# tier4/icp_rust

Hardware: AMD Instinct MI355X
Metric: ICP iterations/sec on 1M-pt 3D pair (higher is better)
Workload: dtype f64

## Files before the change

icp_rust_amd/csrc/api.hip:

```cpp
#include <dlfcn.h>
#include <fcntl.h>
#include <sys/mman.h>
#include <unistd.h>

#include <cfloat>
#include <chrono>
#include <cstdio>
#include <cstring>
#include <atomic>
#include <map>
#include <mutex>
#include <new>

#include "api_internal.hpp"

using namespace icp;
using namespace icp::api;

namespace icp {
namespace api {
int map_hip(hipError_t e) {
  switch (e) {
    case hipSuccess: return ICP_OK;
    case hipErrorOutOfMemory: return ICP_OUT_OF_MEMORY;
    case hipErrorNoDevice:
    case hipErrorInvalidDevice:
    case hipErrorInsufficientDriver:
    case hipErrorNotInitialized: return ICP_NO_DEVICE;
    default: return ICP_HIP_ERROR;
  }
}
}
}

namespace {

template <typename Tp>
hipError_t grow(Tp *&p, size_t count) {
  if (p) {
    hipError_t e = hipFree(p);
    p = nullptr;
    if (e != hipSuccess) return e;
  }
  return hipMalloc(&p, (count ? count : 1) * sizeof(Tp));
}

void free_ctx(GnCtx &c) {
  (void)hipFree(c.d_rx);
  (void)hipFree(c.d_ry);
  (void)hipFree(c.d_hist);
  (void)hipFree(c.d_cand);
  (void)hipFree(c.d_ctl);
  (void)hipFree(c.d_sel);
  (void)hipFree(c.d_scal);
  (void)hipFree(c.d_partials);
  (void)hipFree(c.d_whist);
  (void)hipFree(c.d_wstate);
  (void)hipFree(c.d_wmed);
  (void)hipFree(c.d_wring);
  (void)hipFree(c.d_bkt);
  (void)hipFree(c.d_bkt_dir);
  (void)hipFree(c.d_wjoin);
  if (c.h_res) (void)hipHostFree(c.h_res);
}

void free_workspace(Workspace &w) {
  (void)hipFree(w.d_src);
  (void)hipFree(w.d_a);
  (void)hipFree(w.d_b);
  (void)hipFree(w.d_a2);
  (void)hipFree(w.d_b2);
  (void)hipFree(w.d_a3);
  (void)hipFree(w.d_b3);
  (void)hipFree(w.d_ahead);
  (void)hipFree(w.d_idx);
  (void)hipFree(w.d_idx_slot);
  (void)hipFree(w.d_sa);
  (void)hipFree(w.d_sb);
  if (w.h_whist) (void)hipHostFree(w.h_whist);
  if (w.h_tiny) (void)hipHostFree(w.h_tiny);
  (void)hipFree(w.d_rlist);
  (void)hipFree(w.d_rlist_len);
  (void)hipFree(w.d_part_d);
  (void)hipFree(w.d_part_i);
  free_loop_inbox(w);
  free_loop_plan(w.loop_plan);
  (void)hipFree(w.d_loop_ctl);
  (void)hipFree(w.d_loop_hist);
  (void)hipFree(w.d_loop_part);
  if (w.h_loop_res) (void)hipHostFree(w.h_loop_res);
  free_ctx(w);
  free_ctx(w.alt);
  if (w.spec_stream) {
    (void)hipStreamSynchronize(w.spec_stream);
    (void)hipStreamDestroy(w.spec_stream);
  }
  w = Workspace();
}

hipError_t alloc_ctx(GnCtx &c, hipStream_t s) {
  hipError_t e;
  const size_t hist_bytes = (size_t)kSelRoles * kSelProblems * kSelBins * sizeof(uint32_t);
  if ((e = hipMalloc(&c.d_hist, hist_bytes)) != hipSuccess) return e;
  if ((e = hipMemsetAsync(c.d_hist, 0, hist_bytes, s)) != hipSuccess) return e;
  if ((e = hipMalloc(&c.d_cand, (size_t)2 * kSelProblems * kSelCap * sizeof(unsigned long long))) != hipSuccess) return e;
  if ((e = hipMalloc(&c.d_ctl, sizeof(SelCtl))) != hipSuccess) return e;
  if ((e = hipMemsetAsync(c.d_ctl, 0, sizeof(SelCtl), s)) != hipSuccess) return e;
  if ((e = hipMalloc(&c.d_sel, 2 * kSelProblems * sizeof(SelState))) != hipSuccess) return e;
  if ((e = hipMalloc(&c.d_scal, sizeof(GnScalars))) != hipSuccess) return e;
  if ((e = hipMalloc(&c.d_partials, (size_t)(kTreeMaxBlocks + 1) * (kNSum + 1) * sizeof(double))) != hipSuccess) return e;
  const size_t whist_bytes = ((size_t)2 * kWinBins + kShardStatusWords) * sizeof(uint32_t);
  if ((e = hipMalloc(&c.d_whist, whist_bytes)) != hipSuccess) return e;
  if ((e = hipMemsetAsync(c.d_whist, 0, whist_bytes, s)) != hipSuccess) return e;
  if ((e = hipMalloc(&c.d_wstate, sizeof(WinState))) != hipSuccess) return e;
  if ((e = hipMemsetAsync(c.d_wstate, 0, sizeof(WinState), s)) != hipSuccess) return e;
  if ((e = hipMalloc(&c.d_wmed, (size_t)2 * kWinCapMed * sizeof(double))) != hipSuccess) return e;
  if ((e = hipMalloc(&c.d_wring, (size_t)2 * kWinCapRing * sizeof(double))) != hipSuccess) return e;
  if ((e = hipMalloc(&c.d_bkt, (size_t)kReduceMaxBlocks * kBktStage * sizeof(double))) != hipSuccess) return e;
  if ((e = hipMalloc(&c.d_bkt_dir, (size_t)kReduceMaxBlocks * kBktDir * sizeof(unsigned short))) != hipSuccess) return e;
  if ((e = hipMalloc(&c.d_wjoin, sizeof(WinJoin))) != hipSuccess) return e;
  if ((e = hipMemsetAsync(c.d_wjoin, 0, sizeof(WinJoin), s)) != hipSuccess) return e;
  if ((e = hipHostMalloc(&c.h_res, sizeof(GnResult), hipHostMallocCoherent)) != hipSuccess) return e;
  memset(c.h_res, 0, sizeof(GnResult));
  return hipSuccess;
}

}

namespace icp {

namespace {
using PushFn = int (*)(const char *);
using PopFn = int (*)();
PushFn g_roctx_push = nullptr;
PopFn g_roctx_pop = nullptr;
std::once_flag g_roctx_once;
void roctx_lookup() {
  for (const char *lib : {"librocprofiler-sdk-roctx.so", "librocprofiler-sdk-roctx.so.1", "libroctx64.so", "libroctx64.so.4"}) {
    void *hnd = dlopen(lib, RTLD_LAZY | RTLD_GLOBAL);
    if (!hnd) continue;
    g_roctx_push = reinterpret_cast<PushFn>(dlsym(hnd, "roctxRangePushA"));
    g_roctx_pop = reinterpret_cast<PopFn>(dlsym(hnd, "roctxRangePop"));
    if (g_roctx_push && g_roctx_pop) return;
    g_roctx_push = nullptr;
    g_roctx_pop = nullptr;
  }
}
}
Range::Range(const char *name) {
  std::call_once(g_roctx_once, roctx_lookup);
  if (g_roctx_push) (void)g_roctx_push(name);
}
Range::~Range() {
  if (g_roctx_pop) (void)g_roctx_pop();
}

hipError_t ensure_workspace(icp_handle *h, size_t n, bool need_src) {
  Workspace &w = h->ws;
  hipError_t e;
  if (!w.d_hist) {
    if ((e = alloc_ctx(w, h->stream)) != hipSuccess) return e;
    if ((e = alloc_ctx(w.alt, h->stream)) != hipSuccess) return e;
    int prio_least = 0, prio_greatest = 0;
    (void)hipDeviceGetStreamPriorityRange(&prio_least, &prio_greatest);
    if ((e = hipStreamCreateWithPriority(&w.spec_stream, hipStreamNonBlocking, prio_greatest)) != hipSuccess) return e;
    if ((e = hipMalloc(&w.d_ahead, sizeof(AheadPose))) != hipSuccess) return e;
    if ((e = hipMemsetAsync(w.d_ahead, 0, sizeof(AheadPose), h->stream)) != hipSuccess) return e;
    if ((e = hipStreamSynchronize(h->stream)) != hipSuccess) return e;
  }
  if (n > w.cap_n) {
    if ((e = hipStreamSynchronize(h->stream)) != hipSuccess) return e;
    if ((e = hipStreamSynchronize(w.spec_stream)) != hipSuccess) return e;
    size_t cap = n + n / 8;
    (void)hipFree(w.d_src);
    w.d_src = nullptr;
    if ((e = grow(w.d_a, cap * 2)) != hipSuccess) return e;
    if ((e = grow(w.d_b, cap * 2)) != hipSuccess) return e;
    if ((e = grow(w.d_a2, cap * 2)) != hipSuccess) return e;
    if ((e = grow(w.d_b2, cap * 2)) != hipSuccess) return e;
    if ((e = grow(w.d_a3, cap * 2)) != hipSuccess) return e;
    if ((e = grow(w.d_b3, cap * 2)) != hipSuccess) return e;
    if ((e = grow(w.d_rx, cap)) != hipSuccess) return e;
    if ((e = grow(w.d_ry, cap)) != hipSuccess) return e;
    if ((e = grow(w.alt.d_rx, cap)) != hipSuccess) return e;
    if ((e = grow(w.alt.d_ry, cap)) != hipSuccess) return e;
    if ((e = grow(w.d_idx, cap)) != hipSuccess) return e;
    if ((e = grow(w.d_idx_slot, cap)) != hipSuccess) return e;
    w.cap_n = cap;
  }
  if (need_src && !w.d_src) {
    if ((e = hipMalloc(&w.d_src, (w.cap_n ? w.cap_n : 1) * 3 * sizeof(double))) != hipSuccess) return e;
  }
  return hipSuccess;
}

}

extern "C" const char *icp_status_string(int s) {
  switch (s) {
    case ICP_OK: return "ok";
    case ICP_NONE: return "none (the reference returns None)";
    case ICP_EMPTY_DST: return "empty dst (the reference panics on index.unwrap())";
    case ICP_NAN_INPUT: return "NaN residual (the reference panics on partial_cmp().unwrap())";
    case ICP_BAD_ARGUMENT: return "bad argument";
    case ICP_NO_DEVICE: return "no usable HIP device (there is no CPU fallback)";
    case ICP_HIP_ERROR: return "HIP error";
    case ICP_OUT_OF_MEMORY: return "out of device memory";
    case ICP_RETRY_REPLICATED: return "sharded evaluation: evaluate this one on the gathered pairs";
    case ICP_RETRY_SHARDED: return "sharded evaluation: the window missed; again with the refined window";
    default: return "unknown status";
  }
}

extern "C" int icp_abi_version(void) { return ICP_ABI_VERSION; }

extern "C" int icp_device_pci_bus_id(int device, char out[64]) {
  if (!out) return ICP_BAD_ARGUMENT;
  out[0] = 0;
  if (hipDeviceGetPCIBusId(out, 64, device) != hipSuccess) {
    (void)hipGetLastError();
    return ICP_NO_DEVICE;
  }
  return ICP_OK;
}

extern "C" int icp_device_count(void) {
  int n = 0;
  if (hipGetDeviceCount(&n) != hipSuccess) return 0;
  return n;
}

extern "C" void icp_transform_new(const double p[3], icp_pose *out) { *out = transform_new(p); }
extern "C" void icp_transform_from_rt(const double r[4], const double t[2], icp_pose *out) {
  *out = icp_pose{r[0], r[1], r[2], r[3], t[0], t[1]};
}
extern "C" void icp_transform_identity(icp_pose *out) { *out = transform_identity(); }
extern "C" void icp_transform_apply(const icp_pose *T, const double p[2], double out[2]) {
  double o[2];
  transform_apply(*T, p, o);
  out[0] = o[0];
  out[1] = o[1];
}
extern "C" void icp_transform_inverse(const icp_pose *T, icp_pose *out) { *out = transform_inverse(*T); }
extern "C" void icp_transform_mul(const icp_pose *l, const icp_pose *r, icp_pose *out) {
  *out = transform_mul(*l, *r);
}
extern "C" void icp_se2_exp(const double p[3], double m[9]) { se2_exp(p, m); }
extern "C" void icp_se2_log(const double m[9], double p[3]) { se2_log(m, p); }
// ... 753 lines not shown
          if (on_eval_stream) {
            h->stream = first_stream;
            h->ws.swap_ctx();
          }
          return map_hip(he);
        }
      }
      {
        const int kind_now = it == 0 ? first_kind : (it == 1 ? second_kind : 2);
        if (!(it == 0 && first_pre_launched)) adopt_pool_hint(h->ws, kind_now);
      }
      const int rc = (it == 1 && !hook_first)
                         ? wgn_step(h, d_a, d_b, n, T, delta, &err, [&] { return second_eval_hook(T); }, false, second_kind)
                         : wgn_step(h, d_a, d_b, n, T, delta, &err, it == 0 && first_pre_launched,
                                    it == 0 ? first_kind : (it == 1 ? second_kind : 2));
      if (on_eval_stream) {
        h->stream = first_stream;
        h->ws.swap_ctx();
      }
      if (rc == ICP_NONE) break;
      if (rc != ICP_OK) return rc;
      if ((delta[0] * delta[0] + delta[1] * delta[1]) + delta[2] * delta[2] < ICP_DELTA_NORM_THRESHOLD)
        break;
      if (err > prev_error) break;
      prev_error = err;
      T = transform_mul(transform_new(delta), T);
      ++applied;
    }
  }
  *out = T;
  if (inner_iters) *inner_iters = applied;
  return ICP_OK;
}

extern "C" int icp_estimate_transform_device(icp_handle *h, const double *d_a, const double *d_b, size_t n,
                                             icp_pose *out, uint32_t *inner_iters) {
  if (!h || !out || (n > 0 && (!d_a || !d_b)) || n >= 0xffffffffull) return ICP_BAD_ARGUMENT;
  if (input_size_ok(n)) {
    HIP_TRY(hipSetDevice(h->device));
    HIP_TRY(ensure_workspace(h, n, false));
  }
  return estimate_transform_loop(h, d_a, d_b, n, out, inner_iters, [](const Pose &) { return hipSuccess; });
}

int icp::api::estimate_transform_on_pairs(icp_handle *h, const double *d_a, const double *d_b, size_t n, Pose *out,
                                          uint32_t *inner_iters, int first_kind, int second_kind) {
  return estimate_transform_loop(h, d_a, d_b, n, out, inner_iters, [](const Pose &) { return hipSuccess; }, nullptr,
                                 false, false, first_kind, second_kind);
}

extern "C" int icp_estimate_device(icp_handle *h, const double *d_src, size_t n, const icp_pose *init,
                                   size_t max_iter, icp_pose *out, uint32_t *d_last_idx,
                                   uint32_t *inner_iters) {
  if (!h || !init || !out || (n > 0 && !d_src) || n >= 0xffffffffull) return ICP_BAD_ARGUMENT;
  HIP_TRY(hipSetDevice(h->device));
  HIP_TRY(ensure_workspace(h, n, false));
  struct Quiesce {
    icp_handle *h;
    ~Quiesce() {
      h->ws.bkt_pair_launched = h->ws.alt.bkt_pair_launched = false;
      (void)hipStreamSynchronize(h->stream);
      if (h->ws.spec_stream) (void)hipStreamSynchronize(h->ws.spec_stream);
      h->qsort.valid = false;
      h->qsort.have_prev = false;
      h->qsort.slot_order = false;
    }
  } quiesce_on_exit{h};
  h->qsort.fold_n = 0;
  if (n > 0 && max_iter > 0 && h->m > 0) {
    int tiny_status = -1;
    HIP_TRY(launch_tiny_estimate(h, d_src, n, *init, max_iter, out, d_last_idx, inner_iters, &tiny_status));
    if (tiny_status == 0) {
      ++h->ws.tiny_calls;
      return ICP_OK;
    }
    if (tiny_status == 3) return ICP_NAN_INPUT;
  }
  static const bool no_spec = getenv("ICP_NO_SPECULATION") != nullptr;
  Workspace &w = h->ws;
  const bool loop_ok = gn_loop_applies(n);
  const bool two_streams = !no_spec && h->stream == h->own_stream;
  Pose T = *init;
  if (max_iter > 0) {
    const int prc = icp_prepare_source_device(h, d_src, n, init);
    if (prc != ICP_OK) return prc;
  }
  const bool slot = h->qsort.valid && h->qsort.src == d_src && h->qsort.n == n && (long)n > kGridCoopMaxN;
  h->qsort.slot_order = slot;
  if (slot) h->qsort.fold_n = n;
  uint32_t *const idx_target = slot ? w.d_idx_slot : d_last_idx;
  double *A[3] = {w.d_a, w.d_a2, w.d_a3}, *B[3] = {w.d_b, w.d_b2, w.d_b3};
  int cur = 0;
  bool spec_valid = false, pre_valid = false, first_pre_launched = false;
  const bool can_ahead = two_streams && resolved_nn_mode(h) == ICP_NN_GRID;
  bool ahead_issued = false;
  bool hooked_first = false;
  Pose spec_pose = T;
  uint32_t prev_inner = w.last_inner != 0xffffffffu ? w.last_inner : w.hint_last_inner;
  hipStream_t search_stream = h->stream;
  for (size_t it = 0; it < max_iter; ++it) {
    if (spec_valid && memcmp(&spec_pose, &T, sizeof(Pose)) == 0) {
      cur = (cur + 1) % 3;
      ++w.spec_hits;
      first_pre_launched = pre_valid;
    } else {
      first_pre_launched = false;
      ahead_issued = false;
      if (spec_valid) ++w.spec_misses;
      uint32_t *idx_out = (it + 1 == max_iter && d_last_idx) ? idx_target : nullptr;
      const int rc = icp_correspond_device(h, d_src, n, &T, A[cur], B[cur], idx_out);
      if (rc != ICP_OK) return rc;
    }
    spec_valid = false;
    pre_valid = false;
    const bool device_loop = loop_ok && !first_pre_launched && !(two_streams && prev_inner == 1) && loop_allowed(w);
    const bool speculate = !device_loop && !no_spec && n > 0 && h->m > 0 && it + 1 < max_iter && prev_inner == 1;
    auto launch_spec = [&](const Pose &T1) -> hipError_t {
      spec_pose = transform_mul(T1, T);
      uint32_t *idx_out = (it + 2 == max_iter && d_last_idx) ? idx_target : nullptr;
      const int nxt = (cur + 1) % 3, nxt2 = (cur + 2) % 3;
      spec_valid = true;
      pre_valid = false;
      hipStream_t eval_stream = h->stream;
      h->stream = search_stream;
      hipError_t e = hipSuccess;
      const bool have_search = ahead_issued && w.ahead_seen_valid && memcmp(&w.ahead_seen_pose, &spec_pose, sizeof(Pose)) == 0;
      if (ahead_issued && (have_search || w.ahead_seen_valid)) ++(have_search ? w.ahead_hits : w.ahead_misses);
      ahead_issued = false;
      if (!have_search) e = launch_nn(h, d_src, n, &spec_pose, A[nxt], B[nxt], idx_out);
      if (e == hipSuccess && two_streams) {
        WinParams P;
        w.swap_ctx();
        if (w.gn_dirty) {
          e = launch_sel_init(h, n);
          w.gn_dirty = false;
        }
        if (e == hipSuccess && window_usable(h, n, &P, 0)) {
          ++w.win_tried;
          const bool go_ahead = can_ahead && it + 2 < max_iter;
          WinParams P2;
          const int kind2 = it == 0 ? 4 : 1;
          bool pair = hooked_first && w.bkt_off == 0 && !w.alt.gn_dirty && !w.alt.bkt_pair_launched && bkt_fits(n, P);
          if (pair) {
            adopt_pool_hint(w, kind2);
            pair = window_usable(h, n, &P2, kind2) && bkt_fits(n, P2);
          }
          if (pair) {
            ++w.win_tried;
            e = launch_bkt_pair(h, h->stream, w, A[nxt], B[nxt], P, go_ahead, spec_pose, w.alt, A[cur], B[cur], T1, P2, n);
          } else {
            w.ahead_on = go_ahead;
            w.ahead_outer = spec_pose;
            e = launch_weighted_gn_win(h, A[nxt], B[nxt], n, transform_identity(), P);
            w.ahead_on = false;
          }
          pre_valid = true;
          if (e == hipSuccess && go_ahead) {
            uint32_t *idx_out2 = (it + 3 == max_iter && d_last_idx) ? idx_target : nullptr;
            e = launch_nn_grid_ahead(h, d_src, n, w.d_ahead, A[nxt2], B[nxt2], idx_out2, &ahead_issued);
          }
        }
        w.swap_ctx();
      }
      h->stream = eval_stream;
      return e;
    };
    auto hook = [&](const Pose &T1) -> hipError_t { return speculate ? launch_spec(T1) : hipSuccess; };
// ... 254 lines not shown
```

icp_rust_amd/csrc/common.hpp:

```cpp
#pragma once
#include <hip/hip_runtime.h>

#include <cstddef>
#include <cstdint>
#include <cstdlib>
#include <utility>
#include <vector>

#include "pose.hpp"

namespace icp {


struct Range {
  explicit Range(const char *name);
  ~Range();
  Range(const Range &) = delete;
  Range &operator=(const Range &) = delete;
};

constexpr int kReduceThreads = 512;
constexpr int kReduceMaxBlocks = 256;
constexpr int kTreeMaxBlocks = 2048;
constexpr int kShardMaxWorld = 16;
// ... 68 lines not shown
  unsigned med_cnt[2];
  unsigned ring_inner[2];
  unsigned ring_cnt[2];
  double med_lo[2], med_hi[2];
  double ring_lo[2], ring_hi[2];
  unsigned list_cnt[4][32];
};

struct WinJoinDim {
  double med, sig;
  double tot[10];
  unsigned flags;
  unsigned pad[7];
};
static_assert(sizeof(WinJoinDim) == 128, "a line per dimension");
struct WinJoin {
  unsigned ticket;
  unsigned pad[31];
  WinJoinDim dim[2];
};

struct GnResult {
  double acc[kNAcc + 1];
  double sigma[2];
  double median[2];
  int nan_flag;
  int overflow;
  unsigned seq;
  unsigned pad;
  unsigned status[4];
  Pose next_pose;
  int next_valid;
  int pad2;
};

struct AheadPose {
  Pose T;
  int valid;
  int pad;
};

struct GnCtx {
  double *d_rx = nullptr;
  double *d_ry = nullptr;
  uint32_t *d_hist = nullptr;
  unsigned long long *d_cand = nullptr;
  SelCtl *d_ctl = nullptr;
  SelState *d_sel = nullptr;
  GnScalars *d_scal = nullptr;
  double *d_partials = nullptr;
  GnResult *h_res = nullptr;
  unsigned seq = 0;
  bool gn_dirty = true;
  uint32_t *d_whist = nullptr;
  WinState *d_wstate = nullptr;
  double *d_wmed = nullptr;
  double *d_wring = nullptr;
  double *d_bkt = nullptr;
  unsigned short *d_bkt_dir = nullptr;
  WinJoin *d_wjoin = nullptr;
  bool bkt_pair_launched = false;
};

struct Workspace : GnCtx {
  GnCtx alt;
  void swap_ctx() { std::swap(static_cast<GnCtx &>(*this), alt); }
  size_t cap_n = 0;
  double *d_src = nullptr;
  double *d_a = nullptr;
  double *d_b = nullptr;
  double *d_a2 = nullptr;
  double *d_b2 = nullptr;
  double *d_a3 = nullptr;
  double *d_b3 = nullptr;
  AheadPose *d_ahead = nullptr;
  bool ahead_on = false;
  Pose ahead_outer;
  bool ahead_seen_valid = false;
  Pose ahead_seen_pose;
  unsigned long long ahead_hits = 0, ahead_misses = 0;
  unsigned long long spec_hits = 0, spec_misses = 0;
  uint32_t last_inner = 0xffffffffu;
  hipStream_t spec_stream = nullptr;
  uint32_t *d_idx = nullptr;
  uint32_t *d_idx_slot = nullptr;
  double *d_sa = nullptr, *d_sb = nullptr;
  uint32_t *h_whist = nullptr;
  void *h_tiny = nullptr;
  unsigned long long tiny_calls = 0, tiny_evals = 0, tiny_sorted = 0;
  double *d_rlist = nullptr;
  unsigned *d_rlist_len = nullptr;
  size_t cap_part = 0;
  double *d_part_d = nullptr;
  uint32_t *d_part_i = nullptr;
  bool win_valid = false;
  bool win_wide = false;
  double win_med[2] = {0., 0.}, win_sigma[2] = {0., 0.};
  struct WinPred {
    bool valid = false, wide = false;
    double med[2] = {0., 0.}, sigma[2] = {0., 0.};
  };
  WinPred win_kind[5];
  WinPred hint_kind[5];
  uint32_t hint_last_inner = 0xffffffffu;
  static bool kind_has_slot(int kind) { return kind == 0 || kind == 1 || kind == 3 || kind == 4; }
  unsigned long long win_tried = 0, win_missed = 0, short_evals = 0, radix_evals = 0;
  unsigned long long bkt_evals = 0, bkt_misses = 0;
  unsigned long long fixed_point_skips = 0;
  unsigned bkt_off = 0;
  void *d_loop_ctl = nullptr, *h_loop_res = nullptr;
  uint32_t *d_loop_hist = nullptr;
  double *d_loop_part = nullptr;
  unsigned loop_seq = 0;
  bool loop_off = false;
  unsigned long long loop_launches = 0, loop_evals = 0, loop_handbacks = 0, loop_timeouts = 0;
  void *d_loop_inbox = nullptr;
  int loop_inbox_kind = 0;
  void *loop_inbox_host = nullptr;
  char loop_shm_name[64] = {0};
  unsigned loop_probe_gen = 0;
  unsigned loop_off_calls = 0;
  void *loop_peers[kShardMaxWorld] = {};
  int loop_rank = -1, loop_world = 0;
  void *loop_plan = nullptr;
  unsigned pipe_gen = 0;
  unsigned long long pipe_iters = 0, pipe_handbacks = 0, pipe_gave_up = 0;
  unsigned pipe_off = 0;
};

struct GridParams {
  double lo[3];
  double hi[3];
  double h[3], inv_h[3];
  int n[3];
  int fx;
  double scale;
  float ext;
  int f32_ok;
  float hf[3], ihf[3], nm1f[3];
};

struct GridPoint {
  float x, y, z;
  uint32_t idx;
};

struct Grid {
  bool built = false;
  GridParams p;
  uint32_t ncell = 0;
  uint32_t *d_start = nullptr;
  GridPoint *d_pts = nullptr;
  size_t cap_start = 0, cap_pts = 0;
  uint32_t *t_cell_of = nullptr, *t_cnt = nullptr, *t_btot = nullptr;
  size_t cap_tcell = 0, cap_tcnt = 0, cap_tbtot = 0;
  double *t_part = nullptr;
  uint32_t *d_rcell = nullptr, *d_rcell2 = nullptr, *d_start2 = nullptr, *t_shift = nullptr, *t_cell_new = nullptr;
  GridPoint *d_pts2 = nullptr;
  size_t cap_rcell = 0, cap_rcell2 = 0, cap_start2 = 0, cap_pts2 = 0, cap_shift = 0, cap_cell_new = 0;
  size_t m_full = 0;
  bool rcell_valid = false;
  unsigned long long appends_moved = 0, appends_rebuilt = 0;
  unsigned long long crops_moved = 0, crops_rebuilt = 0;
  uint32_t *d_flag = nullptr;
};

constexpr int kShardStatusWords = 4;
constexpr unsigned kGridPad = 8;

struct ShardCandHeader {
  unsigned cnt[4];
  unsigned fail;
  unsigned pad[11];
};
struct ShardPtrs {
  const unsigned char *p[kShardMaxWorld];
};

struct PrevMatch {
  double x, y, z;
  uint32_t idx, pad;
};

struct QuerySort {
  bool valid = false;
  bool slot_order = false;
  bool identity = false;
  bool presorted = false;
  bool sort_only = false;
  size_t fold_n = 0;
  const double *src = nullptr;
  size_t n = 0, cap = 0;
  uint32_t *d_cell_of = nullptr;
  uint32_t *d_perm = nullptr;
  void *d_tmp = nullptr;
  size_t cap_tmp = 0;
  bool have_prev = false;
  PrevMatch *d_prev = nullptr;
  double *d_sorted = nullptr;
  bool have_certs = false, have_pose = false, have_pose_before = false;
  double decay_r = 0., decay_t = 0.;
  Pose last_pose;
  uint32_t *d_cert_lists = nullptr;
  unsigned *d_cert_ctr = nullptr, *last_cert_ctr = nullptr;
  unsigned cert_seq = 0;
  unsigned long long cert_searches = 0;
};

hipError_t stable_sort_cells(const uint32_t *keys_in, uint32_t *perm_out, unsigned n, unsigned bits, void *&tmp, size_t &cap_tmp,
                             hipStream_t s);

}

struct icp_handle {
  int dim = 0;
  size_t m = 0;
  int device = 0;
  int nn_mode = ICP_NN_AUTO;
  bool single_launch = true;
  bool fixed_point_exit = true;
  bool owns_dst = false;
  const double *d_dst = nullptr;
  double *d_dst_own = nullptr;
  size_t cap_dst_own = 0, cap_soa = 0, cap_f32 = 0;
  double *d_dst_soa = nullptr;
  float *d_dst_f32 = nullptr;
  size_t m_pad = 0;
  bool brute_valid = false;
  bool screen_valid = false;
  hipStream_t own_stream = nullptr;
  hipStream_t stream = nullptr;
  icp::Workspace ws;
  icp::Grid grid;
  icp::QuerySort qsort;
  struct ShardEval {
    icp::WinParams P;
    int kind = 2, rank = 0, world = 1, b0 = 0, b1 = 0, blocks = 0;
    size_t n_local = 0, n_total = 0;
    const double *d_a = nullptr;
    icp::Pose T;
    double *d_ordered = nullptr;
    bool active = false;
    icp::WinParams P2;
    bool refined_ready = false, attempt_refined = false;
  } shard;
  double *d_normals = nullptr;
  size_t cap_normals = 0, normals_m = 0;
  int normals_k = 0;
  void *d_plane_pairs = nullptr;
  double *d_plane_fa = nullptr, *d_plane_fb = nullptr;
  size_t cap_plane = 0;
  int profile = 0;
  unsigned prof_seen = 0;
  std::vector<std::pair<hipEvent_t, hipEvent_t>> prof_events;
  std::vector<std::pair<hipEvent_t, hipEvent_t>> prof_free;
  double *d_dst_alt = nullptr, *d_normals_alt = nullptr;
  size_t cap_dst_alt = 0, cap_normals_alt = 0;
};

namespace icp {

template <typename Tp>
inline hipError_t reserve(Tp *&p, size_t &cap, size_t need) {
  if (need <= cap && p) return hipSuccess;
  if (p) {
    (void)hipFree(p);
    p = nullptr;
    cap = 0;
  }
  const size_t want = need + need / 8 + 1;
  const hipError_t e = hipMalloc(&p, want * sizeof(Tp));
  if (e == hipSuccess) cap = want;
  return e;
}

hipError_t ensure_workspace(icp_handle *h, size_t n, bool need_src);
hipError_t build_target_soa(icp_handle *h);
hipError_t build_target_screen(icp_handle *h);

hipError_t launch_nn_brute(icp_handle *h, const double *d_src, size_t n, const Pose *T,
                           double *d_a, double *d_b, uint32_t *d_idx);

hipError_t launch_materialize(icp_handle *h, const double *d_src, size_t n, const Pose &T, const uint32_t *d_idx,
                              double *d_a, double *d_b);
hipError_t build_grid(icp_handle *h);
hipError_t append_grid(icp_handle *h, size_t m_old, size_t k, bool *done);
hipError_t prepare_queries(icp_handle *h, const double *d_src, size_t n, const Pose &T);
constexpr long kGridCoopMaxN = 65536;
hipError_t launch_unpermute_idx(icp_handle *h, const uint32_t *d_slot_idx, size_t n, uint32_t *d_out);
hipError_t launch_nn_grid(icp_handle *h, const double *d_src, size_t n, const Pose *T, double *d_a,
                          double *d_b, uint32_t *d_idx);
hipError_t launch_nn_grid_ahead(icp_handle *h, const double *d_src, size_t n, const AheadPose *d_pose, double *d_a,
                                double *d_b, uint32_t *d_idx, bool *launched);

hipError_t launch_weighted_gn(icp_handle *h, const double *d_a, const double *d_b, size_t n,
                              const Pose &T);
hipError_t launch_weighted_gn_fast(icp_handle *h, const double *d_a, const double *d_b, size_t n,
                                   const Pose &T);
hipError_t launch_weighted_gn_pull(icp_handle *h, const double *d_a, const double *d_b, size_t n,
                                   const Pose &T);
struct TinyResult {
  Pose pose;
  int status;
  unsigned evals;
  unsigned sorted;
  unsigned pad;
  unsigned long long t[6];
  unsigned long long ts[8];
};
constexpr unsigned kTinyMaxN = 1024, kTinyMaxM = 2048, kTinyMaxIter = 1024;
hipError_t launch_tiny_estimate(icp_handle *h, const double *d_src, size_t n, const Pose &T0, size_t max_iter,
                                Pose *out, uint32_t *d_last_idx, uint32_t *inner_iters, int *status);
struct TinyBatchItem {
  unsigned long long src_first, dst_first, idx_first;
  unsigned n, m;
  unsigned slot, pad;
  Pose init;
};
inline unsigned tiny_threads(size_t n) { return n <= 512 ? 512u : (n <= 768 ? 768u : 1024u); }
size_t tiny_lds_bytes_of(int dim, unsigned m);
hipError_t launch_tiny_estimate_batch(int dim, unsigned threads, unsigned m_max, const double *d_src, const double *d_dst,
                                      const TinyBatchItem *d_items, unsigned count, unsigned max_iter, TinyResult *res,
                                      uint32_t *inner, uint32_t *d_idx, hipStream_t stream, bool *granted);
constexpr int kQualitySums = 6;
struct QualityPart {
  double v[kQualitySums];
  unsigned long long inliers;
  unsigned nan, pad;
};
void quality_clear(size_t n, icp_quality *q);
int quality_result(size_t n, const QualityPart &p, icp_quality *q);
constexpr unsigned kQualityMaxN = 1024, kQualityMaxM = 2048, kQualityBatchThreads = 1024;
struct QualityBatchItem {
  unsigned long long src_first, dst_first;
  unsigned n, m;
  unsigned slot, pad;
  Pose T;
};
hipError_t launch_quality_batch(int dim, unsigned m_max, const double *d_src, const double *d_dst,
                                const QualityBatchItem *d_items, unsigned count, double r2, QualityPart *res,
                                hipStream_t stream);
bool window_usable(const icp_handle *h, size_t n, WinParams *P, int kind = 2, bool any_n = false,
                   double f_override = 0.);
hipError_t launch_weighted_gn_win(icp_handle *h, const double *d_a, const double *d_b, size_t n,
                                  const Pose &T, const WinParams &P);
bool bkt_fits(size_t n, const WinParams &P);
bool bkt_fits_rank(size_t n_total, const WinParams &P);
hipError_t launch_bkt_pair(icp_handle *h, hipStream_t s, GnCtx &first, const double *a1, const double *b1, const WinParams &P1,
                           bool ahead_on, const Pose &ahead_outer, GnCtx &second, const double *a2, const double *b2,
                           const Pose &T2, const WinParams &P2, size_t n);
struct ShardPickRank {
  icp_handle *h;
  int rank, b0, nbl;
  size_t n_local;
  const double *a[2], *b[2];
};
struct ShardPickEval {
  bool alt_ctx;
  Pose T;
  WinParams P;
  bool ahead_on;
  Pose outer;
};
hipError_t launch_shard_evals(const ShardPickRank *rk, int nranks, int world, int B, size_t n_total, unsigned gen0,
                              const ShardPickEval *ev, int nevals);
struct PipeRank {
  icp_handle *h;
  const double *d_src;
  size_t n_local;
  int rank, b0, nbl;
// ... 51 lines not shown
```

icp_rust_amd/csrc/nn_grid.hip:

```cpp
#include "common.hpp"
#include <type_traits>

namespace icp {

__device__ __forceinline__ int cell_coord(double v, double lo, double inv_h, int n) {
  double t = floor((v - lo) * inv_h);
  t = fmin(fmax(t, 0.), (double)(n - 1));
  return (int)t;
}

__global__ void k_grid_bbox(const double *__restrict__ dst, unsigned m, int dim, double *__restrict__ part) {
  __shared__ double smn[3][256], smx[3][256];
  double mn[3], mx[3];
  for (int d = 0; d < 3; ++d) {
    mn[d] = __builtin_huge_val();
    mx[d] = -__builtin_huge_val();
  }
  for (unsigned i = blockIdx.x * 256 + threadIdx.x; i < m; i += gridDim.x * 256)
    for (int d = 0; d < dim; ++d) {
      const double v = dst[(size_t)i * dim + d];
      mn[d] = fmin(mn[d], v);
      mx[d] = fmax(mx[d], v);
    }
  for (int d = 0; d < 3; ++d) {
// ... 1478 lines not shown
  q[2] = DIM == 3 ? src[(size_t)k * DIM + 2] : 0.;
  {
    const double nx = (T.r00 * q[0] + T.r01 * q[1]) + T.tx;
    const double ny = (T.r10 * q[0] + T.r11 * q[1]) + T.ty;
    q[0] = nx;
    q[1] = ny;
  }
  PrevMatch out;
  out.x = out.y = out.z = 0.;
  out.idx = 0xffffffffu;
  out.pad = 0;
  const bool finite = fabs(q[0]) <= 1.7976931348623157e308 && fabs(q[1]) <= 1.7976931348623157e308 &&
                      (DIM < 3 || fabs(q[2]) <= 1.7976931348623157e308);
  if (finite) {
    float qf[3] = {0.f, 0.f, 0.f};
    int c[3] = {0, 0, 0};
#pragma unroll
    for (int d = 0; d < DIM; ++d) {
      qf[d] = (float)(q[d] - g.lo[d]);
      c[d] = (int)fminf(fmaxf(__builtin_floorf(qf[d] * (float)g.inv_h[d]), 0.f), (float)(g.n[d] - 1));
    }
    constexpr int kSeedDiv = 4;
    constexpr uint32_t kSeedBatch = 8;
    const int hx = g.fx > kSeedDiv ? g.fx / kSeedDiv : 1;
    float best = __builtin_huge_valf();
    uint32_t bi = 0xffffffffu, any = 0xffffffffu;
    for (int r = 0;; ++r) {
      const int wx = r * g.fx + hx;
      const int x0 = max(c[0] - wx, 0), x1 = min(c[0] + wx, g.n[0] - 1);
      const int y0 = max(c[1] - r, 0), y1 = min(c[1] + r, g.n[1] - 1);
      const int z0 = DIM == 3 ? max(c[2] - r, 0) : 0, z1 = DIM == 3 ? min(c[2] + r, g.n[2] - 1) : 0;
      for (int iz = z0; iz <= z1; ++iz)
        for (int iy = y0; iy <= y1; ++iy) {
          const uint32_t rb = ((uint32_t)iz * g.n[1] + iy) * g.n[0];
          const uint32_t s0 = start[rb + x0], e0 = start[rb + x1 + 1];
          for (uint32_t j0 = s0; j0 < e0; j0 += kSeedBatch) {
            uint4 wv[kSeedBatch];
#pragma unroll
            for (uint32_t u = 0; u < kSeedBatch; ++u) wv[u] = reinterpret_cast<const uint4 *>(pts)[min(j0 + u, e0 - 1)];
#pragma unroll
            for (uint32_t u = 0; u < kSeedBatch; ++u) {
              const uint4 w = wv[u];
              const float fx = qf[0] - __uint_as_float(w.x), fy = qf[1] - __uint_as_float(w.y);
              const float fz = DIM == 3 ? qf[2] - __uint_as_float(w.z) : 0.f;
              const float s2 = fx * fx + fy * fy + fz * fz;
              if (s2 < best) {
                best = s2;
                bi = w.w;
              } else if (s2 == __builtin_huge_valf() && any == 0xffffffffu && fabsf(__uint_as_float(w.x)) < __builtin_huge_valf() &&
                         fabsf(__uint_as_float(w.y)) < __builtin_huge_valf() && fabsf(__uint_as_float(w.z)) < __builtin_huge_valf()) {
                any = w.w;
              }
            }
          }
        }
      if (bi != 0xffffffffu || any != 0xffffffffu) break;
      if (x0 == 0 && x1 == g.n[0] - 1 && y0 == 0 && y1 == g.n[1] - 1 && z0 == 0 && z1 == (DIM == 3 ? g.n[2] - 1 : 0)) break;
    }
    if (bi == 0xffffffffu) bi = any;
    if (bi != 0xffffffffu) {
      out.x = dst[(size_t)bi * DIM + 0];
      out.y = dst[(size_t)bi * DIM + 1];
      out.z = DIM == 3 ? dst[(size_t)bi * DIM + 2] : 0.;
      out.idx = bi;
    }
  }
  return out;
}

template <int DIM>
__global__ __launch_bounds__(kGridThreads) void k_nn_grid_seeded(const double *__restrict__ src,
                                                                 const uint32_t *__restrict__ perm, unsigned n, Pose T,
                                                                 GridParams g, const uint32_t *__restrict__ start,
                                                                 const GridPoint *__restrict__ pts,
                                                                 const double *__restrict__ dst, uint32_t *__restrict__ idx,
                                                                 double2 *__restrict__ a, double2 *__restrict__ b,
                                                                 PrevMatch *prev) {
  __shared__ CoopLds S;
  const unsigned k = xcd_wave(blockIdx.x, gridDim.x, kXcdChunk) * kGridThreads + threadIdx.x;
  const PrevMatch pm = seed_match<DIM>(k < n ? k : n - 1, src, T, g, start, pts, dst);
  warm_wave<DIM, true>(k, n, src, perm, T, g, start, pts, dst, idx, a, b, prev, pm, S);
}

__global__ void k_query_cell(const double *__restrict__ src, unsigned n, int dim, Pose T, GridParams g, int blk,
                             uint32_t *__restrict__ cell_of, int xshift) {
  const unsigned i = blockIdx.x * blockDim.x + threadIdx.x;
  if (i >= n) return;
  double q[3] = {src[(size_t)i * dim], src[(size_t)i * dim + 1], dim == 3 ? src[(size_t)i * dim + 2] : 0.};
  const double nx = (T.r00 * q[0] + T.r01 * q[1]) + T.tx;
  const double ny = (T.r10 * q[0] + T.r11 * q[1]) + T.ty;
  q[0] = nx;
  q[1] = ny;
  int c[3] = {0, 0, 0};
  for (int d = 0; d < dim; ++d) c[d] = cell_coord(q[d], g.lo[d], g.inv_h[d], g.n[d]);
  c[0] >>= xshift;
  const uint32_t nxk = ((uint32_t)g.n[0] + (1u << xshift) - 1u) >> xshift;
  const uint32_t nyb = ((uint32_t)g.n[1] + (1u << blk) - 1) >> blk, m = (1u << blk) - 1;
  const uint32_t brow = ((uint32_t)c[2] >> blk) * nyb + ((uint32_t)c[1] >> blk);
  const uint32_t sub = (((uint32_t)c[2] & m) << blk) | ((uint32_t)c[1] & m);
  cell_of[i] = ((brow * nxk + (uint32_t)c[0]) << (2 * blk)) | sub;
}

__global__ void k_query_gather(const double *__restrict__ src, unsigned n, int dim, const uint32_t *__restrict__ perm,
                               double *__restrict__ sorted) {
  const size_t c = (size_t)blockIdx.x * blockDim.x + threadIdx.x;
  const size_t tot = (size_t)n * dim;
  const size_t e0 = 2 * c, e1 = e0 + 1;
  if (e0 >= tot) return;
  const size_t k0 = e0 / (unsigned)dim, k1 = e1 / (unsigned)dim;
  const double v0 = src[(size_t)perm[k0] * dim + (e0 - k0 * dim)];
  if (e1 < tot) {
    const double v1 = src[(size_t)perm[k1] * dim + (e1 - k1 * dim)];
    reinterpret_cast<double2 *>(sorted)[c] = make_double2(v0, v1);
  } else {
    sorted[e0] = v0;
  }
}

__global__ void k_unpermute_idx(const uint32_t *__restrict__ slot_idx, const uint32_t *__restrict__ perm, unsigned n,
                                uint32_t *__restrict__ out) {
  const unsigned k = blockIdx.x * blockDim.x + threadIdx.x;
  if (k < n) out[perm[k]] = slot_idx[k];
}

hipError_t launch_unpermute_idx(icp_handle *h, const uint32_t *d_slot_idx, size_t n, uint32_t *d_out) {
  if (n == 0) return hipSuccess;
  hipLaunchKernelGGL(k_unpermute_idx, dim3(((unsigned)n + 255) / 256), dim3(256), 0, h->stream, d_slot_idx,
                     (const uint32_t *)h->qsort.d_perm, (unsigned)n, d_out);
  return hipGetLastError();
}

hipError_t prepare_queries(icp_handle *h, const double *d_src, size_t n_, const Pose &T) {
  Grid &G = h->grid;
  QuerySort &Q = h->qsort;
  Q.valid = false;
  Q.fold_n = 0;
  if (!G.built || n_ == 0) return hipSuccess;
  const unsigned n = (unsigned)n_;
  hipError_t e;
  hipStream_t s = h->stream;
  if (n_ > Q.cap) {
    if ((e = hipStreamSynchronize(s)) != hipSuccess) return e;
    (void)hipFree(Q.d_cell_of);
    (void)hipFree(Q.d_perm);
    (void)hipFree(Q.d_sorted);
    (void)hipFree(Q.d_prev);
    (void)hipFree(Q.d_cert_lists);
    (void)hipFree(Q.d_cert_ctr);
    Q.last_cert_ctr = nullptr;
    Q.d_prev = nullptr;
    Q.d_cert_lists = nullptr;
    Q.d_cert_ctr = nullptr;
    Q.d_cell_of = Q.d_perm = nullptr;
    Q.d_sorted = nullptr;
    Q.cap = 0;
    Q.fold_n = 0;
    if ((e = hipMalloc(&Q.d_cell_of, n_ * 4)) != hipSuccess) return e;
    if ((e = hipMalloc(&Q.d_perm, n_ * 4)) != hipSuccess) return e;
    if ((e = hipMalloc(&Q.d_sorted, n_ * 3 * sizeof(double))) != hipSuccess) return e;
    if ((e = hipMalloc(&Q.d_prev, n_ * sizeof(PrevMatch))) != hipSuccess) return e;
    if ((e = hipMalloc(&Q.d_cert_lists, (n_ + (size_t)(kCertLists + 1) * kCertThreads) * sizeof(uint32_t))) != hipSuccess) return e;
    if ((e = hipMalloc(&Q.d_cert_ctr, (size_t)2 * kCertLists * kCertCtrStride * sizeof(unsigned))) != hipSuccess) return e;
    if ((e = hipMemsetAsync(Q.d_cert_ctr, 0, (size_t)2 * kCertLists * kCertCtrStride * sizeof(unsigned), s)) != hipSuccess) return e;
    Q.cert_seq = 0;
    Q.cap = n_;
  }
  Q.identity = (long)n <= kGridCoopMaxN || Q.presorted;
  Q.presorted = false;
  if (Q.identity) {
    Q.have_prev = false;
    Q.have_certs = false;
    Q.have_pose = Q.have_pose_before = false;
    Q.decay_r = Q.decay_t = 0.;
    Q.src = d_src;
    Q.n = n_;
    Q.valid = true;
    return hipSuccess;
  }
  const unsigned long long keys = (unsigned long long)G.p.n[2] * (unsigned long long)G.p.n[1] * (unsigned long long)G.p.n[0];
  hipLaunchKernelGGL(k_query_cell, dim3((n + 255) / 256), dim3(256), 0, s, d_src, n, h->dim, T, G.p, 0, Q.d_cell_of, 0);
  unsigned bits = 1;
  while (bits < 32 && (1ull << bits) < keys) ++bits;
  if ((e = stable_sort_cells(Q.d_cell_of, Q.d_perm, n, bits, Q.d_tmp, Q.cap_tmp, s)) != hipSuccess) return e;
  if (Q.sort_only) {
    Q.sort_only = false;
    Q.src = d_src;
    Q.n = n_;
    return hipGetLastError();
  }
  {
    const size_t pairs = ((size_t)n * h->dim + 1) / 2;
    hipLaunchKernelGGL(k_query_gather, dim3((unsigned)((pairs + 255) / 256)), dim3(256), 0, s, d_src, n, h->dim,
                       (const uint32_t *)Q.d_perm, Q.d_sorted);
  }
  Q.have_prev = false;
  Q.have_certs = false;
  Q.have_pose = Q.have_pose_before = false;
  Q.decay_r = Q.decay_t = 0.;
  if ((e = hipGetLastError()) != hipSuccess) return e;
  Q.src = d_src;
  Q.n = n_;
  Q.valid = true;
  return hipSuccess;
}

hipError_t launch_nn_grid_ahead(icp_handle *h, const double *d_src, size_t n_, const AheadPose *d_pose, double *d_a,
                                double *d_b, uint32_t *d_idx, bool *launched) {
  *launched = false;
  const Grid &G = h->grid;
  QuerySort &Q = h->qsort;
  if (n_ == 0 || n_ >= 0xffffffffull || !d_pose || h->m == 0 || !G.built || !G.p.f32_ok) return hipSuccess;
  const unsigned n = (unsigned)n_;
  if (!(Q.valid && Q.src == d_src && Q.n == n_ && Q.have_prev)) return hipSuccess;
  const bool coop = (long)n <= kGridCoopMaxN;
  const double *q_src = !Q.identity ? Q.d_sorted : d_src;
  const uint32_t *q_perm = (!Q.slot_order && !Q.identity) ? Q.d_perm : nullptr;
  hipEvent_t ev0 = nullptr, ev1 = nullptr;
  if (h->profile > 0 && (h->prof_seen++ % (unsigned)h->profile) == 0) {
    if (!h->prof_free.empty()) {
      ev0 = h->prof_free.back().first;
      ev1 = h->prof_free.back().second;
      h->prof_free.pop_back();
      (void)hipEventRecord(ev0, h->stream);
    } else if (hipEventCreate(&ev0) == hipSuccess && hipEventCreate(&ev1) == hipSuccess)
      (void)hipEventRecord(ev0, h->stream);
  }
  const unsigned blocks = (unsigned)(((size_t)n * (coop ? 4 : 1) + kGridThreads - 1) / kGridThreads);
  Q.have_pose = false;
  Q.have_certs = false;
  if (coop) {
    if (h->dim == 3)
      hipLaunchKernelGGL((k_nn_grid<3, true, false, 4>), dim3(blocks), dim3(kGridThreads), 0, h->stream, q_src, q_perm, n,
                         transform_identity(), G.p, G.d_start, G.d_pts, h->d_dst, d_idx, (double2 *)d_a, (double2 *)d_b,
                         (const PrevMatch *)Q.d_prev, Q.d_prev, d_pose);
    else
      hipLaunchKernelGGL((k_nn_grid<2, true, false, 4>), dim3(blocks), dim3(kGridThreads), 0, h->stream, q_src, q_perm, n,
                         transform_identity(), G.p, G.d_start, G.d_pts, h->d_dst, d_idx, (double2 *)d_a, (double2 *)d_b,
                         (const PrevMatch *)Q.d_prev, Q.d_prev, d_pose);
  } else if (h->dim == 3)
    hipLaunchKernelGGL(k_nn_grid_warm_coop<3>, dim3(blocks), dim3(kGridThreads), 0, h->stream, q_src, q_perm, n,
                       transform_identity(), G.p, G.d_start, G.d_pts, h->d_dst, d_idx, (double2 *)d_a, (double2 *)d_b, Q.d_prev,
                       (unsigned)kXcdChunk, d_pose);
  else
    hipLaunchKernelGGL(k_nn_grid_warm_coop<2>, dim3(blocks), dim3(kGridThreads), 0, h->stream, q_src, q_perm, n,
                       transform_identity(), G.p, G.d_start, G.d_pts, h->d_dst, d_idx, (double2 *)d_a, (double2 *)d_b, Q.d_prev,
                       (unsigned)kXcdChunk, d_pose);
  const hipError_t e = hipGetLastError();
  if (ev0 && ev1) {
    (void)hipEventRecord(ev1, h->stream);
    h->prof_events.emplace_back(ev0, ev1);
  }
  *launched = e == hipSuccess;
  return e;
}

hipError_t launch_nn_grid(icp_handle *h, const double *d_src, size_t n_, const Pose *Tp, double *d_a,
                          double *d_b, uint32_t *d_idx) {
  if (n_ == 0) return hipSuccess;
  const unsigned n = (unsigned)n_;
  const bool xform = Tp != nullptr;
  const Pose T = xform ? *Tp : transform_identity();
  const Grid &G = h->grid;
  const QuerySort &Q = h->qsort;
  const bool sorted = xform && Q.valid && Q.src == d_src && Q.n == n_;
  const double *q_src = (sorted && !Q.identity) ? Q.d_sorted : d_src;
  const uint32_t *q_perm = (sorted && !Q.slot_order && !Q.identity) ? Q.d_perm : nullptr;
  PrevMatch *q_prev_out = sorted ? Q.d_prev : nullptr;
  const PrevMatch *q_prev = (sorted && Q.have_prev) ? Q.d_prev : nullptr;
  if (sorted) h->qsort.have_prev = true;
  hipEvent_t ev0 = nullptr, ev1 = nullptr;
  if (h->profile > 0 && (h->prof_seen++ % (unsigned)h->profile) == 0) {
    if (!h->prof_free.empty()) {
      ev0 = h->prof_free.back().first;
      ev1 = h->prof_free.back().second;
      h->prof_free.pop_back();
      (void)hipEventRecord(ev0, h->stream);
    } else if (hipEventCreate(&ev0) == hipSuccess && hipEventCreate(&ev1) == hipSuccess)
      (void)hipEventRecord(ev0, h->stream);
  }
  const bool coop = (long)n <= kGridCoopMaxN;
  const unsigned blocks = (unsigned)(((size_t)n * (coop ? 4 : 1) + kGridThreads - 1) / kGridThreads);
  const bool seeded = sorted && !q_prev && !coop && xform && G.p.f32_ok && h->m > 0;
// ... 154 lines not shown
```

Measured before the change: 9890.

## Compute NN seed matches on spec stream concurrently with query sort

On large grid-mode inputs, a new kernel computes initial nearest-neighbor seed matches for every source point on the speculation stream while the main stream sorts queries by cell. After the sort, the main stream waits on an event and gathers the seeds into sorted order as the previous-match buffer, so the first search iteration starts warm. This overlaps seed computation with the sort, at the cost of extra scratch traffic through the a3/b3 buffers and a cross-stream dependency.

```diff
diff --git a/icp_rust_amd/csrc/api.hip b/icp_rust_amd/csrc/api.hip
--- a/icp_rust_amd/csrc/api.hip
+++ b/icp_rust_amd/csrc/api.hip
@@ -95,6 +95,7 @@
     (void)hipStreamSynchronize(w.spec_stream);
     (void)hipStreamDestroy(w.spec_stream);
   }
+  if (w.seed_event) (void)hipEventDestroy(w.seed_event);
   w = Workspace();
 }
 
@@ -164,6 +165,7 @@
     int prio_least = 0, prio_greatest = 0;
     (void)hipDeviceGetStreamPriorityRange(&prio_least, &prio_greatest);
     if ((e = hipStreamCreateWithPriority(&w.spec_stream, hipStreamNonBlocking, prio_greatest)) != hipSuccess) return e;
+    if ((e = hipEventCreateWithFlags(&w.seed_event, hipEventDisableTiming)) != hipSuccess) return e;
     if ((e = hipMalloc(&w.d_ahead, sizeof(AheadPose))) != hipSuccess) return e;
     if ((e = hipMemsetAsync(w.d_ahead, 0, sizeof(AheadPose), h->stream)) != hipSuccess) return e;
     if ((e = hipStreamSynchronize(h->stream)) != hipSuccess) return e;
@@ -1083,7 +1085,18 @@
   const bool two_streams = !no_spec && h->stream == h->own_stream;
   Pose T = *init;
   if (max_iter > 0) {
+    QuerySort &Q = h->qsort;
+    if (two_streams && resolved_nn_mode(h) == ICP_NN_GRID && (long)n > kGridCoopMaxN && h->grid.p.f32_ok && h->m > 0 &&
+        !Q.presorted && !Q.sort_only && w.seed_event) {
+      HIP_TRY(launch_nn_seeds(h, d_src, n, T, w.spec_stream, w.d_a3, w.d_b3));
+      HIP_TRY(hipEventRecord(w.seed_event, w.spec_stream));
+      Q.seed_lo = w.d_a3;
+      Q.seed_hi = w.d_b3;
+      Q.seed_event = w.seed_event;
+    }
     const int prc = icp_prepare_source_device(h, d_src, n, init);
+    Q.seed_lo = Q.seed_hi = nullptr;
+    Q.seed_event = nullptr;
     if (prc != ICP_OK) return prc;
   }
   const bool slot = h->qsort.valid && h->qsort.src == d_src && h->qsort.n == n && (long)n > kGridCoopMaxN;
diff --git a/icp_rust_amd/csrc/common.hpp b/icp_rust_amd/csrc/common.hpp
--- a/icp_rust_amd/csrc/common.hpp
+++ b/icp_rust_amd/csrc/common.hpp
@@ -174,6 +174,7 @@
   unsigned long long spec_hits = 0, spec_misses = 0;
   uint32_t last_inner = 0xffffffffu;
   hipStream_t spec_stream = nullptr;
+  hipEvent_t seed_event = nullptr;
   uint32_t *d_idx = nullptr;
   uint32_t *d_idx_slot = nullptr;
   double *d_sa = nullptr, *d_sb = nullptr;
@@ -289,6 +290,8 @@
   size_t cap_tmp = 0;
   bool have_prev = false;
   PrevMatch *d_prev = nullptr;
+  const void *seed_lo = nullptr, *seed_hi = nullptr;
+  hipEvent_t seed_event = nullptr;
   double *d_sorted = nullptr;
   bool have_certs = false, have_pose = false, have_pose_before = false;
   double decay_r = 0., decay_t = 0.;
@@ -378,6 +381,7 @@
 hipError_t build_grid(icp_handle *h);
 hipError_t append_grid(icp_handle *h, size_t m_old, size_t k, bool *done);
 hipError_t prepare_queries(icp_handle *h, const double *d_src, size_t n, const Pose &T);
+hipError_t launch_nn_seeds(icp_handle *h, const double *d_src, size_t n, const Pose &T, hipStream_t s, void *d_lo, void *d_hi);
 constexpr long kGridCoopMaxN = 65536;
 hipError_t launch_unpermute_idx(icp_handle *h, const uint32_t *d_slot_idx, size_t n, uint32_t *d_out);
 hipError_t launch_nn_grid(icp_handle *h, const double *d_src, size_t n, const Pose *T, double *d_a,
diff --git a/icp_rust_amd/csrc/nn_grid.hip b/icp_rust_amd/csrc/nn_grid.hip
--- a/icp_rust_amd/csrc/nn_grid.hip
+++ b/icp_rust_amd/csrc/nn_grid.hip
@@ -1584,6 +1584,45 @@
   warm_wave<DIM, true>(k, n, src, perm, T, g, start, pts, dst, idx, a, b, prev, pm, S);
 }
 
+#ifndef ICP_SEED_BLOCKS
+#define ICP_SEED_BLOCKS 1024
+#endif
+constexpr int kSeedThreads = 256;
+template <int DIM>
+__global__ __launch_bounds__(kSeedThreads) void k_nn_seeds(const double *__restrict__ src, unsigned n, Pose T, GridParams g,
+                                                           const uint32_t *__restrict__ start,
+                                                           const GridPoint *__restrict__ pts, const double *__restrict__ dst,
+                                                           double2 *__restrict__ lo, uint4 *__restrict__ hi) {
+  for (unsigned i = blockIdx.x * kSeedThreads + threadIdx.x; i < n; i += gridDim.x * kSeedThreads) {
+    const PrevMatch pm = seed_match<DIM>(i, src, T, g, start, pts, dst);
+    lo[i] = make_double2(pm.x, pm.y);
+    hi[i] = make_uint4((uint32_t)__double2loint(pm.z), (uint32_t)__double2hiint(pm.z), pm.idx, pm.pad);
+  }
+}
+
+__global__ void k_seed_gather(const uint4 *__restrict__ lo, const uint4 *__restrict__ hi, const uint32_t *__restrict__ perm,
+                              unsigned n, uint4 *__restrict__ prev) {
+  const size_t c = (size_t)blockIdx.x * blockDim.x + threadIdx.x;
+  if (c >= (size_t)2 * n) return;
+  const uint32_t i = perm[c >> 1];
+  prev[c] = (c & 1u) ? hi[i] : lo[i];
+}
+
+hipError_t launch_nn_seeds(icp_handle *h, const double *d_src, size_t n_, const Pose &T, hipStream_t s, void *d_lo, void *d_hi) {
+  const Grid &G = h->grid;
+  if (n_ == 0 || n_ >= 0xffffffffull || h->m == 0 || !G.built) return hipErrorInvalidValue;
+  const unsigned n = (unsigned)n_;
+  unsigned blocks = (n + kSeedThreads - 1) / kSeedThreads;
+  if (ICP_SEED_BLOCKS > 0 && blocks > (unsigned)ICP_SEED_BLOCKS) blocks = (unsigned)ICP_SEED_BLOCKS;
+  if (h->dim == 3)
+    hipLaunchKernelGGL(k_nn_seeds<3>, dim3(blocks), dim3(kSeedThreads), 0, s, d_src, n, T, G.p, G.d_start, G.d_pts, h->d_dst,
+                       (double2 *)d_lo, (uint4 *)d_hi);
+  else
+    hipLaunchKernelGGL(k_nn_seeds<2>, dim3(blocks), dim3(kSeedThreads), 0, s, d_src, n, T, G.p, G.d_start, G.d_pts, h->d_dst,
+                       (double2 *)d_lo, (uint4 *)d_hi);
+  return hipGetLastError();
+}
+
 __global__ void k_query_cell(const double *__restrict__ src, unsigned n, int dim, Pose T, GridParams g, int blk,
                              uint32_t *__restrict__ cell_of, int xshift) {
   const unsigned i = blockIdx.x * blockDim.x + threadIdx.x;
@@ -1637,6 +1676,10 @@
   QuerySort &Q = h->qsort;
   Q.valid = false;
   Q.fold_n = 0;
+  const void *const seed_lo = Q.seed_lo, *const seed_hi = Q.seed_hi;
+  const hipEvent_t seed_event = Q.seed_event;
+  Q.seed_lo = Q.seed_hi = nullptr;
+  Q.seed_event = nullptr;
   if (!G.built || n_ == 0) return hipSuccess;
   const unsigned n = (unsigned)n_;
   hipError_t e;
@@ -1696,10 +1739,19 @@
                        (const uint32_t *)Q.d_perm, Q.d_sorted);
   }
   Q.have_prev = false;
+  if (seed_lo && seed_hi && seed_event) {
+    if ((e = hipStreamWaitEvent(s, seed_event, 0)) != hipSuccess) return e;
+    hipLaunchKernelGGL(k_seed_gather, dim3((unsigned)(((size_t)2 * n + 255) / 256)), dim3(256), 0, s, (const uint4 *)seed_lo,
+                       (const uint4 *)seed_hi, (const uint32_t *)Q.d_perm, n, reinterpret_cast<uint4 *>(Q.d_prev));
+    Q.have_prev = true;
+  }
   Q.have_certs = false;
   Q.have_pose = Q.have_pose_before = false;
   Q.decay_r = Q.decay_t = 0.;
-  if ((e = hipGetLastError()) != hipSuccess) return e;
+  if ((e = hipGetLastError()) != hipSuccess) {
+    Q.have_prev = false;
+    return e;
+  }
   Q.src = d_src;
   Q.n = n_;
   Q.valid = true;
```

After: 9348. 0.945x the previous value.
